# hanalice/Distributed-ResNet-Tensorflow

Measured on AMD Instinct MI355X. Metric: images/sec (whole node) ResNet-50 bs=128/GPU, higher is better.
Workload: dtype bf16; 1 GPU; model=resnet50_v2_imagenet, global_batch=128, per_gpu_batch=128, image_size=224, num_classes=1001, parallelism=dp1, hip_graph=False, step_mode=plan, wgrad_side_stream=True, fused_stem_pool=True, hw_queues=4

## Files before the change

### csrc/kernels/bn.hip

```cpp
#include "drn_common.h"
#include "drn_conv.h"
#include <stdlib.h>

namespace drn {

__global__ __launch_bounds__(256) void bn_stats_kernel(const bf16_t* __restrict__ x, float* __restrict__ part, int M,
                                                       int C, int rows_per_block, int rep) {
  extern __shared__ __attribute__((aligned(16))) char smem[];
  const int CV = C / 8;
  const int tid = threadIdx.x;
  const int rpp = 256 / CV;
  const int cv = tid % CV;
  const int r0 = tid / CV;
  float s[8], q[8];
#pragma unroll
  for (int j = 0; j < 8; ++j) s[j] = q[j] = 0.f;
  const int mbeg = blockIdx.x * rows_per_block;
  const int mend = min(M, mbeg + rows_per_block);
  if (r0 < rpp) {
    for (int m = mbeg + r0; m < mend; m += rpp) {
      const uint4 v = *reinterpret_cast<const uint4*>(x + (size_t)m * C + cv * 8);
      float f[8];
      unpack8(v, f);
#pragma unroll
// ... 486 lines not shown
    for (int j = 0; j < 8; ++j) {
      f0[j] = f0[j] * sc[j] + sh[j];
      f1[j] = f1[j] * sc[j] + sh[j];
      if (relu) {
        f0[j] = fmaxf(f0[j], 0.f);
        f1[j] = fmaxf(f1[j], 0.f);
      }
    }
    yv[i] = pack8(f0);
    yv[i + stride] = pack8(f1);
  }
  if (i < nvec) {
    float f0[8];
    unpack8(xv[i], f0);
#pragma unroll
    for (int j = 0; j < 8; ++j) {
      f0[j] = f0[j] * sc[j] + sh[j];
      if (relu) f0[j] = fmaxf(f0[j], 0.f);
    }
    yv[i] = pack8(f0);
  }
}

template <bool ADD, bool POOL>
__global__ __launch_bounds__(256) void bn_bwd_apply_fin_kernel(DySrc src, const bf16_t* __restrict__ x,
                                                               const float* __restrict__ scale,
                                                               const float* __restrict__ shift, DrnBnFin f,
                                                               const bf16_t* __restrict__ add, bf16_t* __restrict__ dx,
                                                               int64_t nvec, int C, int relu) {
  extern __shared__ __attribute__((aligned(16))) float lsm[];
  bn_bwd_apply_body<ADD, true, POOL>(src, x, scale, shift, nullptr, nullptr, nullptr, f, add, dx, nvec, C, relu, lsm);
}

static inline int grid_for(int64_t nvec, int per_thread = 1, int cap = 2048) {
  int64_t b = (nvec + 256 * per_thread - 1) / (256 * per_thread);
  if (b > cap) b = cap;
  if (b < 1) b = 1;
  return (int)b;
}

}

static bool pow2(int v) { return v > 0 && (v & (v - 1)) == 0; }

DRN_API int drn_bn_stats_blocks(int M, int C, int rows_per_block) { return (M + rows_per_block - 1) / rows_per_block; }

DRN_API int drn_bn_stats(const void* x, float* part, int M, int C, int rows_per_block, int rep, hipStream_t s) {
  if (C % 8 || C / 8 > 256 || rep < 1) return (int)hipErrorInvalidValue;
  const int G = (M + rows_per_block - 1) / rows_per_block;
  drn::launch(drn::bn_stats_kernel, dim3(G), dim3(256), 256 * 17 * 4, s, (const bf16_t*)x, part, M, C,
                     rows_per_block, rep);
  return (int)hipGetLastError();
}

DRN_API int drn_bn_finalize(float* part, int G, int C, float count, const float* gamma, const float* beta,
                            float eps, float momentum, float* run_mean, float* run_var, float* scale, float* shift,
                            float* mean, float* invstd, hipStream_t s) {
  drn::launch(drn::bn_finalize_kernel, dim3((C + 63) / 64), dim3(256), 0, s, part, G, C, count, gamma, beta,
                     eps, momentum, run_mean, run_var, scale, shift, mean, invstd);
  return (int)hipGetLastError();
}

DRN_API int drn_bn_inference_params(int C, const float* gamma, const float* beta, const float* run_mean,
                                    const float* run_var, float eps, float* scale, float* shift, float* mean,
                                    float* invstd, hipStream_t s) {
  drn::launch(drn::bn_inference_params_kernel, dim3((C + 255) / 256), dim3(256), 0, s, C, gamma, beta,
// ... 41 lines not shown
  if (C % 8 || C / 8 > 256 || rep < 1) return (int)hipErrorInvalidValue;
  const int G = (M + rows_per_block - 1) / rows_per_block;
  drn::DySrc src{(const bf16_t*)dy, dpool, pool_hw};
  drn::launch(drn::bn_bwd_reduce_kernel, dim3(G), dim3(256), 256 * 17 * 4, s, src, (const bf16_t*)x, scale,
                     shift, mean, invstd, part, M, C, rows_per_block, relu, rep);
  return (int)hipGetLastError();
}

DRN_API int drn_bn_finalize_bwd(float* part, int G, int C, float count, const float* gamma,
                                const float* invstd, float* dgamma, float* dbeta, float* coef, hipStream_t s) {
  drn::launch(drn::bn_finalize_bwd_kernel, dim3((C + 63) / 64), dim3(256), 0, s, part, G, C, count, gamma,
                     invstd, dgamma, dbeta, coef);
  return (int)hipGetLastError();
}

static bool fin_ok(const DrnBnFin* f, int C) {
  return f != nullptr && f->stats != nullptr && f->G >= 1 && f->G <= DRN_BN_FIN_GMAX && f->C == C &&
         f->count > 0.f && f->gamma != nullptr;
}

DRN_API int drn_bn_fin_fwd_launch(const DrnBnFin* f, hipStream_t s) {
  if (!fin_ok(f, f ? f->C : 0) || f->beta == nullptr || f->scale == nullptr || f->shift == nullptr ||
      f->mean == nullptr || f->invstd == nullptr)
    return (int)hipErrorInvalidValue;
  drn::launch(drn::bn_fin_fwd_kernel, dim3((f->C + 255) / 256), dim3(256), 0, s, *f);
  return (int)hipGetLastError();
}

DRN_API int drn_bn_apply_fin(const void* x, void* y, const DrnBnFin* f, int64_t M, int C, int relu, hipStream_t s) {
  if (C % 8 || !pow2(C / 8) || C / 8 > 256 || !fin_ok(f, C) || f->beta == nullptr ||
      (f->publish && (f->scale == nullptr || f->shift == nullptr || f->mean == nullptr || f->invstd == nullptr)))
    return (int)hipErrorInvalidValue;
  const int64_t nvec = M * (C / 8);
  drn::launch(drn::bn_apply_fin_kernel, dim3(drn::grid_for(nvec, 2)), dim3(256), 2 * C * sizeof(float), s,
                     (const bf16_t*)x, (bf16_t*)y, *f, nvec, C / 8, relu);
  return (int)hipGetLastError();
}

DRN_API int drn_bn_bwd_apply_fin(const void* dy, const float* dpool, int pool_hw, const void* x, const float* scale,
                                 const float* shift, const DrnBnFin* f, const void* add, void* dx, int64_t M, int C,
                                 int relu, hipStream_t s) {
  if (C % 8 || !pow2(C / 8) || C / 8 > 256 || !fin_ok(f, C) || f->mean == nullptr || f->invstd == nullptr ||
      (f->publish && (f->dgamma == nullptr || f->dbeta == nullptr)))
    return (int)hipErrorInvalidValue;
  const int64_t nvec = M * (C / 8);
  if (nvec >= (int64_t(1) << 31)) return (int)hipErrorInvalidValue;
  drn::DySrc src{(const bf16_t*)dy, dpool, pool_hw};
  const dim3 grid(drn::grid_for(nvec, 4, 1024));
  const size_t lds = 3 * C * sizeof(float);
#define DRN_BWD_FIN(ADD, POOL)                                                                                     \
  drn::launch((drn::bn_bwd_apply_fin_kernel<ADD, POOL>), grid, dim3(256), lds, s, src, (const bf16_t*)x, scale, \
                     shift, *f, (const bf16_t*)add, (bf16_t*)dx, nvec, C, relu)
  if (pool_hw > 0) {
    if (add != nullptr) DRN_BWD_FIN(true, true);
    else DRN_BWD_FIN(false, true);
  } else {
    if (add != nullptr) DRN_BWD_FIN(true, false);
    else DRN_BWD_FIN(false, false);
  }
#undef DRN_BWD_FIN
  return (int)hipGetLastError();
}

DRN_API int drn_bn_fin_size() { return (int)sizeof(DrnBnFin); }
DRN_API int drn_conv_args_size() { return (int)sizeof(DrnConvFwdArgs); }
DRN_API int drn_wgrad_args_size() { return (int)sizeof(DrnConvWgradArgs); }

DRN_API int drn_bn_bwd_apply(const void* dy, const float* dpool, int pool_hw, const void* x, const float* scale,
                             const float* shift, const float* mean, const float* invstd, const float* coef,
                             const void* add, void* dx, int64_t M, int C, int relu, hipStream_t s) {
  if (C % 8 || !pow2(C / 8) || C / 8 > 256) return (int)hipErrorInvalidValue;
  const int64_t nvec = M * (C / 8);
  if (nvec >= (int64_t(1) << 31)) return (int)hipErrorInvalidValue;
  drn::DySrc src{(const bf16_t*)dy, dpool, pool_hw};
  const dim3 grid(drn::grid_for(nvec, 4, 1024));
#define DRN_BWD(ADD, POOL)                                                                                         \
  drn::launch((drn::bn_bwd_apply_kernel<ADD, POOL>), grid, dim3(256), 0, s, src, (const bf16_t*)x, scale, shift, \
                     mean, invstd, coef, (const bf16_t*)add, (bf16_t*)dx, nvec, C, relu)
  if (pool_hw > 0) {
    if (add != nullptr) DRN_BWD(true, true);
    else DRN_BWD(false, true);
  } else {
    if (add != nullptr) DRN_BWD(true, false);
    else DRN_BWD(false, false);
  }
// ... 4 lines not shown
```

### csrc/kernels/head.hip

```cpp
#include "drn_common.h"

namespace drn {

__global__ __launch_bounds__(256) void bnrelu_pool_kernel(const bf16_t* __restrict__ x, const float* __restrict__ scale,
                                                          const float* __restrict__ shift, float* __restrict__ pooled,
                                                          int HW, int C, int relu) {
  const int n = blockIdx.x;
  const int CV = C / 8;
  for (int cv = threadIdx.x; cv < CV; cv += blockDim.x) {
    const int c = cv * 8;
    float acc[8], sc[8], sh[8];
#pragma unroll
    for (int j = 0; j < 8; ++j) {
      acc[j] = 0.f;
      sc[j] = scale ? scale[c + j] : 1.f;
      sh[j] = scale ? shift[c + j] : 0.f;
    }
    for (int hw = 0; hw < HW; ++hw) {
      float f[8];
      unpack8(*reinterpret_cast<const uint4*>(x + ((size_t)n * HW + hw) * C + c), f);
#pragma unroll
      for (int j = 0; j < 8; ++j) {
        float v = f[j] * sc[j] + sh[j];
        if (relu) v = fmaxf(v, 0.f);
        acc[j] += v;
      }
    }
    const float inv = 1.f / (float)HW;
#pragma unroll
    for (int j = 0; j < 8; ++j) pooled[(size_t)n * C + c + j] = acc[j] * inv;
  }
}

__global__ __launch_bounds__(256) void sgemm_kernel(int ta, int tb, int M, int N, int K, float alpha,
                                                    const float* __restrict__ A, int lda,
                                                    const float* __restrict__ B, int ldb, float beta,
                                                    float* __restrict__ Cm, int ldc, const float* __restrict__ bias) {
  constexpr int BM = 64, BN = 64, BK = 32;
  constexpr int LA = BK * BM / 256, LB = BK * BN / 256;
  __shared__ float As[2][BK][BM + 1];
  __shared__ float Bs[2][BK][BN + 1];
  const int tid = threadIdx.x, lane = tid & 63, wave = tid >> 6;
  const int m0 = blockIdx.y * BM, n0 = blockIdx.x * BN;
  const int wm = (wave & 1) * 32, wn = (wave >> 1) * 32;
  const int ksz = (((K + gridDim.z - 1) / gridDim.z) + BK - 1) / BK * BK;
  const int kb = blockIdx.z * ksz, ke = min(K, kb + ksz);
  if (gridDim.z > 1) {
    Cm += (size_t)blockIdx.z * M * ldc;
    beta = 0.f;
    bias = nullptr;
    alpha = 1.f;
  }
  f32x4_t acc[2][2];
#pragma unroll
  for (int i = 0; i < 2; ++i)
#pragma unroll
// ... 331 lines not shown
  const int cl = threadIdx.x & 31, sl = threadIdx.x >> 5;
  const int j = blockIdx.x * 32 + cl;
  float s0 = 0.f, s1 = 0.f, s2 = 0.f, s3 = 0.f;
  if (j < cols) {
    int n = sl;
    for (; n + 24 < rows; n += 32) {
      s0 += in[(size_t)n * cols + j];
      s1 += in[(size_t)(n + 8) * cols + j];
      s2 += in[(size_t)(n + 16) * cols + j];
      s3 += in[(size_t)(n + 24) * cols + j];
    }
    for (; n < rows; n += 8) s0 += in[(size_t)n * cols + j];
  }
  red[sl][cl] = (s0 + s1) + (s2 + s3);
  __syncthreads();
  if (sl == 0 && j < cols) {
    float s = 0.f;
#pragma unroll
    for (int k = 0; k < 8; ++k) s += red[k][cl];
    out[j] = accumulate ? out[j] + scale * s : scale * s;
  }
}

}

DRN_API int drn_bnrelu_pool(const void* x, const float* scale, const float* shift, float* pooled, int N, int HW,
                            int C, int relu, hipStream_t s) {
  if (C % 8) return (int)hipErrorInvalidValue;
  drn::launch(drn::bnrelu_pool_kernel, dim3(N), dim3(256), 0, s, (const bf16_t*)x, scale, shift, pooled, HW, C,
                     relu);
  return (int)hipGetLastError();
}

DRN_API int drn_sgemm(int ta, int tb, int M, int N, int K, float alpha, const float* A, int lda, const float* B,
                      int ldb, float beta, float* C, int ldc, const float* bias, int splits, float* ws,
                      hipStream_t s) {
  if (splits < 1 || (splits > 1 && ws == nullptr)) return (int)hipErrorInvalidValue;
  dim3 grid((N + 63) / 64, (M + 63) / 64, splits);
  drn::launch(drn::sgemm_kernel, grid, dim3(256), 0, s, ta, tb, M, N, K, alpha, A, lda, B, ldb, beta,
                     splits > 1 ? ws : C, ldc, bias);
  if (splits > 1)
    drn::launch(drn::sgemm_finish_kernel, dim3((M * N + 255) / 256), dim3(256), 0, s, ws, splits, M, N, ldc,
                       alpha, beta, C, bias);
  return (int)hipGetLastError();
}

DRN_API int drn_softmax_xent(const float* logits, const int* labels, int N, int ncls, float grad_scale,
                             float* dlogits, float* loss, float* probs, int* correct, hipStream_t s) {
  drn::launch(drn::softmax_xent_kernel, dim3(N), dim3(256), 0, s, logits, labels, ncls, grad_scale, dlogits,
                     loss, probs, correct);
  return (int)hipGetLastError();
}

DRN_API int drn_softmax_xent_ex(const float* logits, const int* labels, int N, int ncls, float grad_scale,
                                float smoothing, int top_k, float* dlogits, float* loss, float* probs, int* correct,
                                int* correct_k, hipStream_t s) {
  if (!(smoothing >= 0.f && smoothing < 1.f) || top_k < 1 || N < 1 || ncls < 1) return (int)hipErrorInvalidValue;
  auto kern = ncls <= 256 * drn::XENT_REG_ROW ? drn::softmax_xent_ex_kernel<true> : drn::softmax_xent_ex_kernel<false>;
  drn::launch(kern, dim3(N), dim3(256), 0, s, logits, labels, ncls, grad_scale, smoothing, top_k, dlogits, loss,
                     probs, correct, correct_k);
  return (int)hipGetLastError();
}

DRN_API int drn_softmax_xent_mix(const float* logits, const int* labels, const void* table, int N, int ncls,
                                 float grad_scale, float smoothing, int top_k, float* dlogits, float* loss,
                                 float* probs, int* correct, int* correct_k, hipStream_t s) {
// ... 14 lines not shown
```

### distributed_resnet_tensorflow_amd/ops/_lib.py

```python
from __future__ import annotations

import ctypes
import os
import threading
from pathlib import Path

import torch

_LIB = None
_LOCK = threading.Lock()
LIB_PATH = Path(os.environ.get("DRN_KERNEL_LIB") or Path(__file__).resolve().parent / "libdrn_kernels.so")
_OPTIONAL = {"drn_conv_trace_set", "drn_wgrad_trace_set"}

c_int = ctypes.c_int
c_i64 = ctypes.c_int64
c_f = ctypes.c_float
c_p = ctypes.c_void_p


class DrnFastDiv(ctypes.Structure):
    _fields_ = [("d", ctypes.c_uint32), ("m", ctypes.c_uint32), ("s", ctypes.c_uint32), ("pad_", ctypes.c_uint32)]

    @classmethod
    def make(cls, d: int) -> "DrnFastDiv":
# ... 47 lines not shown


def conv_cfg_info(cfg: int):
    info = DrnConvCfgInfo()
    return info if lib().drn_conv_cfg_info(int(cfg), ctypes.byref(info)) == 0 else None


_SIGS = {
    "drn_version": ([], c_int),
    "drn_conv_fwd": ([ctypes.POINTER(DrnConvFwdArgs), c_p], c_int),
    "drn_conv_fwd_tiles_p": ([c_int, c_int], c_int),
    "drn_conv_fwd2": ([ctypes.POINTER(DrnConvFwdArgs), c_p, c_p], c_int),
    "drn_conv_glds_ok": ([ctypes.POINTER(DrnConvFwdArgs)], c_int),
    "drn_conv_glds_num_cfgs": ([], c_int),
    "drn_conv_trace_set": ([c_p], c_int),
    "drn_wgrad_trace_set": ([c_p], c_int),
    "drn_conv_glds_default_cfg": ([ctypes.POINTER(DrnConvFwdArgs)], c_int),
    "drn_conv_wgrad": ([ctypes.POINTER(DrnConvWgradArgs), c_p], c_int),
    "drn_conv_wgrad2": ([ctypes.POINTER(DrnConvWgradArgs), c_p, c_int, c_p], c_int),
    "drn_splitk_reduce": ([c_p, c_p, c_i64, c_int, c_f, c_int, c_p], c_int),
    "drn_bn_stats": ([c_p, c_p, c_int, c_int, c_int, c_int, c_p], c_int),
    "drn_bn_finalize": ([c_p, c_int, c_int, c_f, c_p, c_p, c_f, c_f, c_p, c_p, c_p, c_p, c_p, c_p, c_p], c_int),
    "drn_bn_inference_params": ([c_int, c_p, c_p, c_p, c_p, c_f, c_p, c_p, c_p, c_p, c_p], c_int),
    "drn_bn_apply": ([c_p, c_p, c_p, c_p, c_i64, c_int, c_int, c_p], c_int),
    "drn_bn_apply_stats": ([c_p, c_p, c_p, c_f, c_p, c_p, c_f, c_f, c_p, c_p, c_p, c_p, c_p, c_p, c_i64, c_int,
                            c_int, c_p], c_int),
    "drn_bn_bwd_apply_stats": ([c_p, c_p, c_int, c_p, c_p, c_p, c_p, c_p, c_p, c_f, c_p, c_p, c_p, c_p, c_p, c_i64,
                                c_int, c_int, c_p], c_int),
    "drn_bn_bwd_reduce": ([c_p, c_p, c_int, c_p, c_p, c_p, c_p, c_p, c_p, c_int, c_int, c_int, c_int, c_int, c_p],
                          c_int),
    "drn_bn_finalize_bwd": ([c_p, c_int, c_int, c_f, c_p, c_p, c_p, c_p, c_p, c_p], c_int),
    "drn_bn_bwd_apply": ([c_p, c_p, c_int, c_p, c_p, c_p, c_p, c_p, c_p, c_p, c_p, c_i64, c_int, c_int, c_p], c_int),
    "drn_bnrelu_pool": ([c_p, c_p, c_p, c_p, c_int, c_int, c_int, c_int, c_p], c_int),
    "drn_sgemm": ([c_int, c_int, c_int, c_int, c_int, c_f, c_p, c_int, c_p, c_int, c_f, c_p, c_int, c_p, c_int, c_p,
                   c_p], c_int),
    "drn_softmax_xent": ([c_p, c_p, c_int, c_int, c_f, c_p, c_p, c_p, c_p, c_p], c_int),
    "drn_softmax_xent_ex": ([c_p, c_p, c_int, c_int, c_f, c_f, c_int, c_p, c_p, c_p, c_p, c_p, c_p], c_int),
    "drn_softmax_xent_mix": ([c_p, c_p, c_p, c_int, c_int, c_f, c_f, c_int, c_p, c_p, c_p, c_p, c_p, c_p], c_int),
    "drn_mix_pairs": ([c_p, c_p, c_p, c_int, c_int, c_int, c_p], c_int),
    "drn_mix_rec_size": ([], c_int),
    "drn_colsum": ([c_p, c_int, c_int, c_p, c_f, c_int, c_p], c_int),
    "drn_maxpool_fwd": ([c_p, c_p, c_p] + [c_int] * 10 + [c_p, c_int, c_p], c_int),
    "drn_maxpool_bwd": ([c_p, c_p, c_p] + [c_int] * 10 + [c_p], c_int),
    "drn_sgd_momentum": ([c_p, c_p, c_p, c_int, c_p, c_i64, c_p, c_f, c_f, c_f, c_p, c_p], c_int),
    "drn_lars_momentum": ([c_p, c_p, c_p, c_int, c_p, c_p, c_int, c_int, c_p, c_p, c_p, c_f, c_f, c_f, c_f, c_f,
                           c_p, c_p], c_int),
    "drn_sgd_momentum_ema": ([c_p, c_p, c_p, c_int, c_p, c_i64, c_p, c_f, c_f, c_f, c_p, c_p, c_p, c_p], c_int),
    "drn_lars_momentum_ema": ([c_p, c_p, c_p, c_int, c_p, c_p, c_int, c_int, c_p, c_p, c_p, c_f, c_f, c_f, c_f, c_f,
                               c_p, c_p, c_p, c_p], c_int),
    "drn_lars_slot_size": ([], c_int),
    "drn_lars_chunk": ([], c_int),
    "drn_cast_bf16": ([c_p, c_p, c_i64, c_p], c_int),
    "drn_stem_pack_input": ([c_p, c_p, c_int, c_int, c_p], c_int),
    "drn_stem_pack_weights": ([c_p, c_p, c_int, c_int, c_int, c_int, c_int, c_int, c_p], c_int),
    "drn_stem_unpack_grad": ([c_p, c_p, c_int, c_int, c_int, c_int, c_int, c_int, c_p], c_int),
    "drn_stem_conv_pool": ([c_p, c_p, c_p, c_p, c_p] + [c_int] * 11 + [c_p], c_int),
    "drn_weight_tflip": ([c_p, c_p, c_p, c_int, c_i64, c_p], c_int),
    "drn_fill_f32": ([c_p, c_i64, c_f, c_p], c_int),
    "drn_cifar_augment": ([c_p, c_p, c_p, c_int, c_int, c_int, c_int, c_p], c_int),
    "drn_vgg_preprocess": ([c_p, c_p, c_p, c_int, c_int, c_int, c_f, c_f, c_f, c_p], c_int),
    "drn_p2p_signal": ([c_p, c_int, c_p], c_int),
    "drn_p2p_reduce": ([c_p, c_int, c_int, c_p], c_int),
    "drn_p2p_reduce2": ([c_p, c_int, c_int, c_p], c_int),
    "drn_p2p_step": ([c_p, c_p, c_p], c_int),
    "drn_p2p_cast": ([c_p, c_p, c_i64, c_p], c_int),
    "drn_p2p_args_size": ([], c_int),
# ... 91 lines not shown
```

### distributed_resnet_tensorflow_amd/ops/backend.py

```python
from __future__ import annotations

import ctypes
import os
from dataclasses import dataclass
from typing import Optional

import numpy as np
import torch
import torch.nn.functional as F

from . import _lib


@dataclass(frozen=True)
class ConvGeom:
    stride: int = 1
    pad_h: int = 0
    pad_w: int = 0
    dil: int = 1


def _ptr(t):
    return None if t is None else t.data_ptr()

# ... 170 lines not shown
    @staticmethod
    def conv_stats_tiles(M, K):
        return 1

    def bn_apply_stats(self, x, y, acc, count, gamma, beta, run_mean, run_var, scale, shift, mean, invstd,
                       momentum, eps, relu=True):
        self.bn_finalize(acc.clone(), 1, count, gamma, beta, run_mean, run_var, scale, shift, mean, invstd,
                         momentum, eps, update_running=True)
        self.bn_apply(x, y, scale, shift, relu=relu)

    def bn_bwd_apply_stats(self, dy, dpool, pool_hw, x, scale, shift, mean, invstd, acc, count, gamma, dgamma,
                           dbeta, add, dx, coef, relu=True):
        self.bn_finalize_bwd(acc.clone(), 1, count, gamma, invstd, dgamma, dbeta, coef)
        self.bn_bwd_apply(dy, dpool, pool_hw, x, scale, shift, mean, invstd, coef, add, dx, relu=relu)


    def fill_(self, t, v: float):
        t.fill_(v)

    @staticmethod
    def _check_out_fill(y, residual, out_map, bn_bwd):
        assert out_map is not None and bn_bwd is None and residual is None, "out_fill: plain strided output only"
        assert out_map.P * out_map.stride >= y.shape[1] and out_map.Q * out_map.stride >= y.shape[2], \
            "out_fill: the phase grid's sibling positions do not cover the output"

    def _publish_fwd(self, f: BnCfin):
        self.bn_finalize(f.stats, f.G, f.count, f.gamma, f.beta, f.run_mean, f.run_var, f.scale, f.shift, f.mean,
                         f.invstd, f.momentum, f.eps, update_running=f.run_mean is not None)

    def bn_apply_fin(self, x, y, fin: BnCfin, relu=True):
        if fin.publish:
            self._publish_fwd(fin)
        self.bn_apply(x, y, fin.scale, fin.shift, relu=relu)

    def bn_bwd_apply_fin(self, dy, dpool, pool_hw, x, scale, shift, fin: BnCfin, add, dx, relu=True):
        C = fin.C
        coef = torch.empty(3 * C, dtype=fin.gamma.dtype, device=x.device)
        dg = fin.dgamma if fin.publish else torch.empty_like(fin.gamma)
        db = fin.dbeta if fin.publish else torch.empty_like(fin.gamma)
        self.bn_finalize_bwd(fin.stats, fin.G, fin.count, fin.gamma, fin.invstd, dg, db, coef)
        self.bn_bwd_apply(dy, dpool, pool_hw, x, scale, shift, fin.mean, fin.invstd, coef, add, dx, relu=relu)


WGRAD_PIPELINES = "0,2,3,4,5,6,7,8,9,10"


class HipBackend(_Common):
    name = "hip"
    act_dtype = torch.bfloat16
    acc_dtype = torch.float32
    stats_replicas = 8

    def __init__(self, device="cuda"):
        self.device = torch.device(device)
        self.L = _lib.lib()
        self.zero_page = torch.zeros(1024, dtype=torch.float32, device=self.device)
        self.conv_cfg: dict = {}
        self.ks_ws = torch.zeros(1, dtype=torch.float32, device=self.device)
        self.ks_tickets = torch.zeros(1 << 16, dtype=torch.int32, device=self.device)
        self.KS_FACTORS = (2, 3, 4)
        self.SK_BLOCKS = (256, 512)
        self.forced_cfg = None
        self.autotune = os.environ.get("DRN_AUTOTUNE", "1") == "1"
        self.wgrad_ns: dict = {}
        self.wgrad_atomic_ok = False
        self.wgrad_atomic_used = False
        self.forced_wgrad_ns = None
        self.tune_log: list = []
        self._db = None
        self.db_hits = 0
        self.tune_iters = int(os.environ.get("DRN_TUNE_ITERS", "5"))
        self.tune_top = int(os.environ.get("DRN_TUNE_TOP", "4"))
        self.tune_rounds = int(os.environ.get("DRN_TUNE_ROUNDS", "2"))
        self._fin_bufs: dict = {}
        self.conv_cands: dict = {}
        self._insitu = None
        self.recording = False

    def _timed(self, launch, n: int) -> float:
        ev0, ev1 = torch.cuda.Event(enable_timing=True), torch.cuda.Event(enable_timing=True)
        ev0.record()
        for _ in range(n):
            launch()
        ev1.record()
        ev1.synchronize()
        return ev0.elapsed_time(ev1) / n

    def tune_db(self):
        if self._db is None:
            from .tunedb import TuneDB, section_for
            self._db = TuneDB(section_for(self.device, self.L))
        return self._db

    def save_tune_db(self) -> bool:
        return self._db is not None and self._db.save()

    def stream(self):
        return torch.cuda.current_stream(self.device).cuda_stream

    def conv_args(self, x, w, y, g: ConvGeom, in_bn=None, relu_in=True, residual=None, stats=None, out_map=None,
                  bn_bwd=None, bn_fin: Optional[BnFin] = None, in_fin: Optional[BnCfin] = None):
        N, H, W, C = x.shape
        K, R, S, C2 = w.shape
        N2, P, Q, K2 = y.shape
        oH, oW = P, Q
        if out_map is not None:
            P, Q = out_map.P, out_map.Q
# ... 365 lines not shown
    def bn_inference(self, gamma, beta, run_mean, run_var, eps, scale, shift, mean=None, invstd=None):
        _lib.check(self.L.drn_bn_inference_params(gamma.numel(), gamma.data_ptr(), beta.data_ptr(),
                                                  run_mean.data_ptr(), run_var.data_ptr(), eps, scale.data_ptr(),
                                                  shift.data_ptr(), _ptr(mean), _ptr(invstd), self.stream()),
                   "drn_bn_inference_params")

    def bn_apply(self, x, y, scale, shift, relu=True):
        C = x.shape[-1]
        _lib.check(self.L.drn_bn_apply(x.data_ptr(), y.data_ptr(), scale.data_ptr(), shift.data_ptr(),
                                       x.numel() // C, C, 1 if relu else 0, self.stream()), "drn_bn_apply")

    def bn_apply_stats(self, x, y, acc, count, gamma, beta, run_mean, run_var, scale, shift, mean, invstd,
                       momentum, eps, relu=True):
        C = x.shape[-1]
        _aligned16(acc, gamma, beta, run_mean, run_var, scale, shift, mean, invstd)
        _lib.check(self.L.drn_bn_apply_stats(x.data_ptr(), y.data_ptr(), acc.data_ptr(), float(count),
                                             gamma.data_ptr(), beta.data_ptr(), float(eps), float(momentum),
                                             run_mean.data_ptr(), run_var.data_ptr(), scale.data_ptr(),
                                             shift.data_ptr(), mean.data_ptr(), invstd.data_ptr(), x.numel() // C, C,
                                             1 if relu else 0, self.stream()), "drn_bn_apply_stats")

    def bn_bwd_apply_stats(self, dy, dpool, pool_hw, x, scale, shift, mean, invstd, acc, count, gamma, dgamma,
                           dbeta, add, dx, coef=None, relu=True):
        C = x.shape[-1]
        _aligned16(acc, gamma, dgamma, dbeta, scale, shift, mean, invstd)
        _lib.check(self.L.drn_bn_bwd_apply_stats(_ptr(dy), _ptr(dpool), pool_hw, x.data_ptr(), scale.data_ptr(),
                                                 shift.data_ptr(), mean.data_ptr(), invstd.data_ptr(),
                                                 acc.data_ptr(), float(count), gamma.data_ptr(), dgamma.data_ptr(),
                                                 dbeta.data_ptr(), _ptr(add), dx.data_ptr(), x.numel() // C, C,
                                                 1 if relu else 0, self.stream()), "drn_bn_bwd_apply_stats")

    def bn_apply_fin(self, x, y, fin: BnCfin, relu=True):
        C = x.shape[-1]
        if C >= self.BN_FIN_SPLIT_C and fin.publish:
            self.bn_finalize(fin.stats, fin.G, fin.count, fin.gamma, fin.beta, fin.run_mean, fin.run_var, fin.scale,
                             fin.shift, fin.mean, fin.invstd, fin.momentum, fin.eps,
                             update_running=fin.run_mean is not None)
            self.bn_apply(x, y, fin.scale, fin.shift, relu=relu)
            return
        f = fin.struct()
        _lib.check(self.L.drn_bn_apply_fin(x.data_ptr(), y.data_ptr(), ctypes.byref(f), x.numel() // C, C,
                                           1 if relu else 0, self.stream()), "drn_bn_apply_fin")

    BN_FIN_SPLIT_C = 1024

    def _fin_scratch(self, C: int) -> torch.Tensor:
        buf = self._fin_bufs.get(C)
        if buf is None:
            buf = self._fin_bufs[C] = torch.empty(5 * C, dtype=torch.float32, device=self.device)
        return buf

    def bn_bwd_apply_fin(self, dy, dpool, pool_hw, x, scale, shift, fin: BnCfin, add, dx, relu=True):
        C = x.shape[-1]
        _aligned16(scale, shift)
        if C >= self.BN_FIN_SPLIT_C:
            buf = self._fin_scratch(C)
            coef = buf[:3 * C]
            dg = fin.dgamma if fin.publish else buf[3 * C:4 * C]
            db = fin.dbeta if fin.publish else buf[4 * C:]
            self.bn_finalize_bwd(fin.stats, fin.G, fin.count, fin.gamma, fin.invstd, dg, db, coef)
            self.bn_bwd_apply(dy, dpool, pool_hw, x, scale, shift, fin.mean, fin.invstd, coef, add, dx, relu=relu)
            return
        f = fin.struct()
        _lib.check(self.L.drn_bn_bwd_apply_fin(_ptr(dy), _ptr(dpool), pool_hw, x.data_ptr(), scale.data_ptr(),
                                               shift.data_ptr(), ctypes.byref(f), _ptr(add), dx.data_ptr(),
                                               x.numel() // C, C, 1 if relu else 0, self.stream()),
                   "drn_bn_bwd_apply_fin")

    def bn_bwd_reduce(self, dy, dpool, pool_hw, x, scale, shift, mean, invstd, part, relu=True):
        C = x.shape[-1]
        M = x.numel() // C
        rpb = self.bn_rows_per_block(M, C)
        _lib.check(self.L.drn_bn_bwd_reduce(_ptr(dy), _ptr(dpool), pool_hw, x.data_ptr(), scale.data_ptr(),
                                            shift.data_ptr(), mean.data_ptr(), invstd.data_ptr(), part.data_ptr(),
                                            M, C, rpb, 1 if relu else 0, part.numel() // (2 * C), self.stream()),
                   "drn_bn_bwd_reduce")
        return part.numel() // (2 * C)

    def bn_finalize_bwd(self, part, G, count, gamma, invstd, dgamma, dbeta, coef):
        _lib.check(self.L.drn_bn_finalize_bwd(part.data_ptr(), G, gamma.numel(), float(count), gamma.data_ptr(),
                                              invstd.data_ptr(), dgamma.data_ptr(), dbeta.data_ptr(),
                                              coef.data_ptr(), self.stream()), "drn_bn_finalize_bwd")

    def bn_bwd_apply(self, dy, dpool, pool_hw, x, scale, shift, mean, invstd, coef, add, dx, relu=True):
        C = x.shape[-1]
        _lib.check(self.L.drn_bn_bwd_apply(_ptr(dy), _ptr(dpool), pool_hw, x.data_ptr(), scale.data_ptr(),
                                           shift.data_ptr(), mean.data_ptr(), invstd.data_ptr(), coef.data_ptr(),
                                           _ptr(add), dx.data_ptr(), x.numel() // C, C, 1 if relu else 0,
                                           self.stream()), "drn_bn_bwd_apply")

    def pool_bnrelu(self, x, scale, shift, pooled, relu=True):
        N, H, W, C = x.shape
        _lib.check(self.L.drn_bnrelu_pool(x.data_ptr(), _ptr(scale), _ptr(shift), pooled.data_ptr(), N, H * W, C,
                                          1 if relu else 0, self.stream()), "drn_bnrelu_pool")

    _sgemm_ws: dict = {}
    _retired_ws: list = []
    SGEMM_TARGET_WG = 256

    def sgemm(self, ta, tb, M, N, K, alpha, A, lda, B, ldb, beta, C, ldc, bias=None):
        tiles = ((M + 63) // 64) * ((N + 63) // 64)
        splits = max(1, min(K // 128, self.SGEMM_TARGET_WG // max(tiles, 1)))
        ws = None
        if splits > 1:
            need = splits * M * ldc
            key = (C.device, self.stream())
            ws = HipBackend._sgemm_ws.get(key)
            if ws is None or ws.numel() < need:
                if ws is not None:
                    if torch.cuda.is_current_stream_capturing():
                        raise RuntimeError("sgemm workspace must be sized before graph capture")
                    HipBackend._retired_ws.append(ws)
                ws = torch.empty(max(need, 1 << 20), dtype=torch.float32, device=C.device)
                HipBackend._sgemm_ws[key] = ws
        _lib.check(self.L.drn_sgemm(int(ta), int(tb), M, N, K, float(alpha), A.data_ptr(), lda, B.data_ptr(), ldb,
                                    float(beta), C.data_ptr(), ldc, _ptr(bias), splits, _ptr(ws), self.stream()),
                   "drn_sgemm")

    def softmax_xent(self, logits, labels, grad_scale, dlogits, loss, correct, probs=None):
        N, ncls = logits.shape
        _lib.check(self.L.drn_softmax_xent(logits.data_ptr(), labels.data_ptr(), N, ncls, float(grad_scale),
                                           _ptr(dlogits), loss.data_ptr(), _ptr(probs), _ptr(correct),
                                           self.stream()), "drn_softmax_xent")

    def softmax_xent_ex(self, logits, labels, grad_scale, dlogits, loss, correct, probs=None, smoothing=0.0, top_k=1,
                        correct_k=None):
        N, ncls = logits.shape
# ... 599 lines not shown
```

### distributed_resnet_tensorflow_amd/runtime/executor.py

```python
from __future__ import annotations

import contextlib
import os

from dataclasses import dataclass
from typing import Callable, List, Optional

import torch

from ..models.spec import Block, BN, Conv, NetSpec
from ..ops.backend import BnCfin, ConvGeom, OutMap, dgrad_geom, tflip_desc, tflip_table
from .params import ParamStore

BN_DECAY = 0.997
BN_EPSILON = 1e-5


@dataclass
class BNState:
    bn: BN
    gamma: torch.Tensor
    beta: torch.Tensor
    dgamma: torch.Tensor
    dbeta: torch.Tensor
# ... 154 lines not shown
                        Hph = (in_hw - ph + st - 1) // st
                        Wph = (in_hw - pw + st - 1) // st
                        if not rs or not ss or Hph <= 0 or Wph <= 0:
                            full = False
                            continue
                        r0, s0 = max(rs), max(ss)
                        dmin_h, dmin_w = (ph + p - r0) // st, (pw + p - s0) // st
                        wt_descs.append(tflip_desc(s.offset, wt_off, K, R, R, C, Ru=len(rs), Sv=len(ss),
                                                   r0=r0, s0=s0, dr=-st, ds=-st))
                        phases.append(DgradPhase((C, len(rs), len(ss), K), wt_off,
                                                 ConvGeom(1, -dmin_h, -dmin_w, 1), OutMap(Hph, Wph, st, ph, pw)))
                        wt_off += C * len(rs) * len(ss) * K
        op = ConvOp(c, g, P.compute_w(name), phases, P.g(name), s.offset, full)
        return op, wt_off

    def _bn_shapes(self):
        sp, N = self.spec, self.N
        hs = sp.stem_hw
        out = [(N * hs * hs, sp.stem.cout)]
        if sp.maxpool:
            out.append((N * sp.pool_hw * sp.pool_hw, sp.stem.cout))
        for blk in sp.blocks:
            hw = blk.in_hw
            out.append((N * hw * hw, blk.in_c))
            for b, c in zip(blk.bns, blk.convs[:-1]):
                hw = c.out_hw(hw)
                out += [(N * hw * hw, c.cout)] * 2
            out.append((N * blk.out_hw * blk.out_hw, blk.out_c))
        out.append((N * sp.blocks[-1].out_hw ** 2, sp.final_c))
        return out

    def _det_replicas(self, M: int, C: int) -> int:
        return max(((M + 63) // 64) * ((C + 63) // 64), 1024)

    def _reps(self, C: int) -> int:
        r = max(1, min(self.stats_rep, self.stats_rep * 256 // C))
        return min(r, 8) if self.cfin else r

    def _stats_for(self, M: int, C: int) -> tuple[torch.Tensor, int]:
        R = self._det_replicas(M, C) if self.deterministic else self._reps(C)
        n = (2 * C * R + 15) // 16 * 16
        if self._arena_off + n > self._arena_cap:
            raise RuntimeError("statistics arena exhausted")
        t = self.stats_arena[self._arena_off:self._arena_off + 2 * C * R].view(R, 2, C)
        self._arena_off += n
        return t, R

    def all_bn_states(self) -> List[BNState]:
        return [b for bp in self.blocks for b in bp.bn] + [self.final_bn]

    def _alloc(self):
        sp, N = self.spec, self.N
        be = self.be
        all_c = [b.c for blk in sp.blocks for b in [blk.bn1] + list(blk.bns)] + [sp.final_bn.c, sp.stem.cout]
        self.stats_rep = int(getattr(be, "stats_replicas", 1))
        if self.deterministic:
            arena = 64 + sum(2 * ((2 * c * self._det_replicas(m, c) + 15) // 16 * 16) for m, c in self._bn_shapes())
        else:
            arena = sum(2 * ((2 * c * self._reps(c) + 15) // 16 * 16) for c in all_c) + 64
        self._arena_cap = arena
        self.stats_arena = self._f32(arena)
        self._arena_off = 0
        wt_descs, wt_off = [], 0
        self.stem_op, wt_off = self._conv_op(sp.stem, wt_descs, wt_off)
        self._stem_hi = int(self.stem_op.dw.numel()) if self.stem_op.grad_lo == 0 else 0
        stem_macs = N * sp.stem_hw * sp.stem_hw * sp.stem.cout * sp.stem.k * sp.stem.k * sp.stem.cin_store
# ... 222 lines not shown

    def forward(self, train: bool = True):
        be, sp = self.be, self.spec
        if train:
            be.zero_(self.stats_arena)
        st = self.stem_op
        if self.stem_pool:
            be.stem_pack_input(self.images, self.stem_xp)
            fused = train and not self.deterministic
            img = sp.image_size
            be.stem_conv_pool(self.stem_xp, self.stem_w4, self.pool_out, self.pool_arg, self.stem_geom4, img, img,
                              sp.stem_hw, sp.stem_hw, stats=self.pool_stats if fused else None)
            if train and not fused:
                be.bn_stats(self.pool_out, self.pool_stats)
        elif self.stem_pack:
            be.stem_pack_input(self.images, self.stem_xp)
            be.conv_fwd(self.stem_xp, self.stem_w4, self.stem_out, self.stem_geom4,
                        stats=self.stem_stats if train else None)
        else:
            be.conv_fwd(self.images, st.w, self.stem_out, st.geom, stats=self.stem_stats if train else None)
        if sp.maxpool and not self.stem_pool:
            ph = sp.pool_hw
            pad = max((ph - 1) * 2 + 3 - sp.stem_hw, 0) // 2
            fused = train and not self.deterministic
            be.maxpool_fwd(self.stem_out, self.pool_out, self.pool_arg, 3, 2, pad, pad,
                           stats=self.pool_stats if fused else None)
            if train and not fused:
                be.bn_stats(self.pool_out, self.pool_stats)
        for bp in self.blocks:
            self._block_fwd(bp, train)
            if self.check_nan:
                self._check(bp.out, f"forward output of block {bp.blk.stage}.{bp.blk.index}")
        fb = self.final_bn
        self._bn_fwd(fb, train)
        be.pool_bnrelu(self.last_out, fb.scale, fb.shift, self.pooled, relu=True)
        N, C, ncls = self.N, sp.final_c, sp.num_classes
        be.sgemm(0, 1, N, ncls, C, 1.0, self.pooled, C, self.dense_w, C, 0.0, self.logits, ncls, bias=self.dense_b)
        smoothing = self.label_smoothing if train else 0.0
        if self.mix and train:
            be.softmax_xent_mix(self.logits, self.labels, self.mix_table, 1.0 / N, self.dlogits, self.loss_vec,
                                self.correct, smoothing=smoothing, top_k=max(self.top_k, 1),
                                correct_k=self.correct_k)
        elif smoothing == 0.0 and self.top_k < 2:
            be.softmax_xent(self.logits, self.labels, 1.0 / N, self.dlogits if train else None, self.loss_vec,
                            self.correct)
        else:
            be.softmax_xent_ex(self.logits, self.labels, 1.0 / N, self.dlogits if train else None, self.loss_vec,
                               self.correct, smoothing=smoothing, top_k=max(self.top_k, 1),
                               correct_k=self.correct_k)
        if self.check_nan:
            self._check(self.loss_vec, "cross-entropy")

    def set_mix(self, table):
        if self.mix_table is None:
            raise RuntimeError("this executor does not mix (Executor(mix=False))")
        from ..ops.backend import mix_table_tensor
        t = mix_table_tensor(table)
        if tuple(t.shape) != (self.N, 8):
            raise ValueError(f"the mix table has {t.shape[0]} records, the batch {self.N} samples")
        self.mix_table.copy_(t, non_blocking=True)

    def _check(self, t: torch.Tensor, what: str):
        if not bool(torch.isfinite(t.float()).all()):
            raise FloatingPointError(f"non-finite values in {what}")

    def check_gradients(self):
        bad = [s.name for s in self.P.slots
               if not bool(torch.isfinite(self.P.grad[s.offset:s.offset + s.numel]).all())]
# ... 407 lines not shown
```

Before: 13350 images/sec.

## Slice fused BN-finalize kernels by channel and fuse finalize into final pool

Adds channel-sliced variants of the fused BN-finalize apply and backward-apply kernels for C>256. Each block finalizes only a 256-channel slice in shared memory, so wide layers no longer go through separate finalize and apply launches. Also fuses the final BN's finalize into the global-average-pool+ReLU head kernel, removing a separate BN forward step. The trade-off is redundant finalize work across blocks: every row-block recomputes the statistics reduction for its slice, and the pool kernel recomputes it per image.

```diff
diff --git a/csrc/kernels/bn.hip b/csrc/kernels/bn.hip
--- a/csrc/kernels/bn.hip
+++ b/csrc/kernels/bn.hip
@@ -542,6 +542,138 @@
   bn_bwd_apply_body<ADD, true, POOL>(src, x, scale, shift, nullptr, nullptr, nullptr, f, add, dx, nvec, C, relu, lsm);
 }
 
+constexpr int kFinSlice = 256;
+
+struct BnSlice {
+  uint32_t i0, stride;
+  int c0, cl;
+};
+__device__ __forceinline__ BnSlice bn_slice(int C) {
+  constexpr int SV = kFinSlice / 8, ROWS = 256 / SV;
+  const int CV = C / 8;
+  const int sv = threadIdx.x % SV, r = threadIdx.x / SV;
+  BnSlice s;
+  s.c0 = blockIdx.y * kFinSlice;
+  s.cl = sv * 8;
+  s.i0 = (blockIdx.x * ROWS + r) * CV + blockIdx.y * SV + sv;
+  s.stride = gridDim.x * ROWS * CV;
+  return s;
+}
+
+__global__ __launch_bounds__(256) void bn_apply_fin_sliced_kernel(const bf16_t* __restrict__ x,
+                                                                  bf16_t* __restrict__ y, DrnBnFin f, int64_t nvec,
+                                                                  int CV, int relu) {
+  __shared__ __attribute__((aligned(16))) float lsm[2 * kFinSlice];
+  const BnSlice sl = bn_slice(CV * 8);
+  {
+    const int t = fin_slot(threadIdx.x);
+    drn_bn_fin_fwd(f, sl.c0 + threadIdx.x, f.publish && blockIdx.x == 0, lsm[t], lsm[kFinSlice + t]);
+  }
+  __syncthreads();
+  float sc[8], sh[8];
+  load8f_fin(lsm, sl.cl, sc);
+  load8f_fin(lsm + kFinSlice, sl.cl, sh);
+  const int64_t stride = sl.stride;
+  const uint4* xv = reinterpret_cast<const uint4*>(x);
+  uint4* yv = reinterpret_cast<uint4*>(y);
+  int64_t i = sl.i0;
+  for (; i + stride < nvec; i += 2 * stride) {
+    const uint4 v0 = xv[i], v1 = xv[i + stride];
+    float f0[8], f1[8];
+    unpack8(v0, f0);
+    unpack8(v1, f1);
+#pragma unroll
+    for (int j = 0; j < 8; ++j) {
+      f0[j] = f0[j] * sc[j] + sh[j];
+      f1[j] = f1[j] * sc[j] + sh[j];
+      if (relu) {
+        f0[j] = fmaxf(f0[j], 0.f);
+        f1[j] = fmaxf(f1[j], 0.f);
+      }
+    }
+    yv[i] = pack8(f0);
+    yv[i + stride] = pack8(f1);
+  }
+  if (i < nvec) {
+    float f0[8];
+    unpack8(xv[i], f0);
+#pragma unroll
+    for (int j = 0; j < 8; ++j) {
+      f0[j] = f0[j] * sc[j] + sh[j];
+      if (relu) f0[j] = fmaxf(f0[j], 0.f);
+    }
+    yv[i] = pack8(f0);
+  }
+}
+
+template <bool ADD, bool POOL>
+__global__ __launch_bounds__(256) void bn_bwd_apply_fin_sliced_kernel(DySrc src, const bf16_t* __restrict__ x,
+                                                                      const float* __restrict__ scale,
+                                                                      const float* __restrict__ shift, DrnBnFin f,
+                                                                      const bf16_t* __restrict__ add,
+                                                                      bf16_t* __restrict__ dx, int64_t nvec, int C,
+                                                                      int relu) {
+  __shared__ __attribute__((aligned(16))) float lsm[3 * kFinSlice];
+  constexpr int U = 4;
+  const int cv_shift = __ffs(C / 8) - 1;
+  const uint32_t n = (uint32_t)nvec;
+  const BnSlice sl = bn_slice(C);
+  const uint32_t stride = sl.stride, i0 = sl.i0;
+  const int c = sl.c0 + sl.cl;
+  const uint4* __restrict__ xg = reinterpret_cast<const uint4*>(x);
+  const uint4* __restrict__ dg = reinterpret_cast<const uint4*>(src.dy);
+  const uint4* __restrict__ ag = reinterpret_cast<const uint4*>(add);
+  uint4* __restrict__ og = reinterpret_cast<uint4*>(dx);
+  const uint32_t safe = i0 < n ? i0 : 0;
+  uint4 xr[U], dr[U], ar[U];
+  auto load = [&](uint32_t base) {
+#pragma unroll
+    for (int u = 0; u < U; ++u) {
+      const uint32_t i = base + u * stride < n ? base + u * stride : safe;
+      xr[u] = xg[i];
+      if constexpr (!POOL) dr[u] = dg[i];
+      if constexpr (ADD) ar[u] = ag[i];
+    }
+  };
+  load(i0);
+  float sc[8], sh[8], A[8], B[8], D[8];
+  load8f(scale + c, sc);
+  load8f(shift + c, sh);
+  {
+    const int t = fin_slot(threadIdx.x);
+    drn_bn_fin_bwd(f, sl.c0 + threadIdx.x, f.publish && blockIdx.x == 0, lsm[t], lsm[kFinSlice + t],
+                   lsm[2 * kFinSlice + t]);
+  }
+  __syncthreads();
+  load8f_fin(lsm, sl.cl, A);
+  load8f_fin(lsm + kFinSlice, sl.cl, B);
+  load8f_fin(lsm + 2 * kFinSlice, sl.cl, D);
+  for (uint32_t base = i0; base < n; base += U * stride) {
+    uint4 o[U];
+#pragma unroll
+    for (int u = 0; u < U; ++u) {
+      float fd[8];
+      if constexpr (POOL) src.load_vec(base + u * stride < n ? base + u * stride : safe, cv_shift, C, c, fd);
+      else unpack8(dr[u], fd);
+      bn_bwd_fin_vec<ADD>(xr[u], fd, ar[u], A, B, D, sc, sh, relu);
+      o[u] = pack8(fd);
+    }
+#pragma unroll
+    for (int u = 0; u < U; ++u)
+      if (base + u * stride < n) og[base + u * stride] = o[u];
+    if (base + U * stride < n) load(base + U * stride);
+  }
+}
+
+static inline dim3 sliced_grid(int64_t M, int C, int per_thread, int cap) {
+  const int gy = C / kFinSlice;
+  const int rows = 256 / (kFinSlice / 8) * per_thread;
+  int64_t gx = (M + rows - 1) / rows;
+  if (gx > cap / gy) gx = cap / gy;
+  if (gx < 1) gx = 1;
+  return dim3((unsigned)gx, (unsigned)gy);
+}
+
 static inline int grid_for(int64_t nvec, int per_thread = 1, int cap = 2048) {
   int64_t b = (nvec + 256 * per_thread - 1) / (256 * per_thread);
   if (b > cap) b = cap;
@@ -649,6 +781,12 @@
       (f->publish && (f->scale == nullptr || f->shift == nullptr || f->mean == nullptr || f->invstd == nullptr)))
     return (int)hipErrorInvalidValue;
   const int64_t nvec = M * (C / 8);
+  if (C > drn::kFinSlice) {
+    if (nvec >= (int64_t(1) << 31)) return (int)hipErrorInvalidValue;
+    drn::launch(drn::bn_apply_fin_sliced_kernel, drn::sliced_grid(M, C, 2, 2048), dim3(256), 0, s, (const bf16_t*)x,
+                (bf16_t*)y, *f, nvec, C / 8, relu);
+    return (int)hipGetLastError();
+  }
   drn::launch(drn::bn_apply_fin_kernel, dim3(drn::grid_for(nvec, 2)), dim3(256), 2 * C * sizeof(float), s,
                      (const bf16_t*)x, (bf16_t*)y, *f, nvec, C / 8, relu);
   return (int)hipGetLastError();
@@ -665,9 +803,17 @@
   drn::DySrc src{(const bf16_t*)dy, dpool, pool_hw};
   const dim3 grid(drn::grid_for(nvec, 4, 1024));
   const size_t lds = 3 * C * sizeof(float);
+  const bool sliced = C > drn::kFinSlice;
+  const dim3 sgrid = sliced ? drn::sliced_grid(M, C, 4, 1024) : grid;
 #define DRN_BWD_FIN(ADD, POOL)                                                                                     \
-  drn::launch((drn::bn_bwd_apply_fin_kernel<ADD, POOL>), grid, dim3(256), lds, s, src, (const bf16_t*)x, scale, \
-                     shift, *f, (const bf16_t*)add, (bf16_t*)dx, nvec, C, relu)
+  do {                                                                                                             \
+    if (sliced)                                                                                                    \
+      drn::launch((drn::bn_bwd_apply_fin_sliced_kernel<ADD, POOL>), sgrid, dim3(256), 0, s, src,                  \
+                  (const bf16_t*)x, scale, shift, *f, (const bf16_t*)add, (bf16_t*)dx, nvec, C, relu);             \
+    else                                                                                                           \
+      drn::launch((drn::bn_bwd_apply_fin_kernel<ADD, POOL>), grid, dim3(256), lds, s, src, (const bf16_t*)x,      \
+                  scale, shift, *f, (const bf16_t*)add, (bf16_t*)dx, nvec, C, relu);                               \
+  } while (0)
   if (pool_hw > 0) {
     if (add != nullptr) DRN_BWD_FIN(true, true);
     else DRN_BWD_FIN(false, true);
diff --git a/csrc/kernels/head.hip b/csrc/kernels/head.hip
--- a/csrc/kernels/head.hip
+++ b/csrc/kernels/head.hip
@@ -1,4 +1,5 @@
 #include "drn_common.h"
+#include "drn_conv.h"
 
 namespace drn {
 
@@ -22,6 +23,35 @@
 #pragma unroll
       for (int j = 0; j < 8; ++j) {
         float v = f[j] * sc[j] + sh[j];
+        if (relu) v = fmaxf(v, 0.f);
+        acc[j] += v;
+      }
+    }
+    const float inv = 1.f / (float)HW;
+#pragma unroll
+    for (int j = 0; j < 8; ++j) pooled[(size_t)n * C + c + j] = acc[j] * inv;
+  }
+}
+
+__global__ __launch_bounds__(256) void bnrelu_pool_fin_kernel(const bf16_t* __restrict__ x, DrnBnFin f,
+                                                              float* __restrict__ pooled, int HW, int C, int relu) {
+  const int n = blockIdx.x;
+  const int CV = C / 8;
+  const bool pub = f.publish && blockIdx.x == 0;
+  for (int cv = threadIdx.x; cv < CV; cv += blockDim.x) {
+    const int c = cv * 8;
+    float acc[8], sc[8], sh[8];
+#pragma unroll
+    for (int j = 0; j < 8; ++j) {
+      acc[j] = 0.f;
+      drn_bn_fin_fwd(f, c + j, pub, sc[j], sh[j]);
+    }
+    for (int hw = 0; hw < HW; ++hw) {
+      float v8[8];
+      unpack8(*reinterpret_cast<const uint4*>(x + ((size_t)n * HW + hw) * C + c), v8);
+#pragma unroll
+      for (int j = 0; j < 8; ++j) {
+        float v = v8[j] * sc[j] + sh[j];
         if (relu) v = fmaxf(v, 0.f);
         acc[j] += v;
       }
@@ -419,6 +449,16 @@
   return (int)hipGetLastError();
 }
 
+DRN_API int drn_bnrelu_pool_fin(const void* x, const DrnBnFin* f, float* pooled, int N, int HW, int C, int relu,
+                                hipStream_t s) {
+  if (C % 8 || N < 1 || f == nullptr || f->stats == nullptr || f->G < 1 || f->G > DRN_BN_FIN_GMAX || f->C != C ||
+      !(f->count > 0.f) || f->gamma == nullptr || f->beta == nullptr ||
+      (f->publish && (f->scale == nullptr || f->shift == nullptr || f->mean == nullptr || f->invstd == nullptr)))
+    return (int)hipErrorInvalidValue;
+  drn::launch(drn::bnrelu_pool_fin_kernel, dim3(N), dim3(256), 0, s, (const bf16_t*)x, *f, pooled, HW, C, relu);
+  return (int)hipGetLastError();
+}
+
 DRN_API int drn_sgemm(int ta, int tb, int M, int N, int K, float alpha, const float* A, int lda, const float* B,
                       int ldb, float beta, float* C, int ldc, const float* bias, int splits, float* ws,
                       hipStream_t s) {
diff --git a/distributed_resnet_tensorflow_amd/ops/_lib.py b/distributed_resnet_tensorflow_amd/ops/_lib.py
--- a/distributed_resnet_tensorflow_amd/ops/_lib.py
+++ b/distributed_resnet_tensorflow_amd/ops/_lib.py
@@ -103,6 +103,7 @@
     "drn_bn_finalize_bwd": ([c_p, c_int, c_int, c_f, c_p, c_p, c_p, c_p, c_p, c_p], c_int),
     "drn_bn_bwd_apply": ([c_p, c_p, c_int, c_p, c_p, c_p, c_p, c_p, c_p, c_p, c_p, c_i64, c_int, c_int, c_p], c_int),
     "drn_bnrelu_pool": ([c_p, c_p, c_p, c_p, c_int, c_int, c_int, c_int, c_p], c_int),
+    "drn_bnrelu_pool_fin": ([c_p, c_p, c_p, c_int, c_int, c_int, c_int, c_p], c_int),
     "drn_sgemm": ([c_int, c_int, c_int, c_int, c_int, c_f, c_p, c_int, c_p, c_int, c_f, c_p, c_int, c_p, c_int, c_p,
                    c_p], c_int),
     "drn_softmax_xent": ([c_p, c_p, c_int, c_int, c_f, c_p, c_p, c_p, c_p, c_p], c_int),
diff --git a/distributed_resnet_tensorflow_amd/ops/backend.py b/distributed_resnet_tensorflow_amd/ops/backend.py
--- a/distributed_resnet_tensorflow_amd/ops/backend.py
+++ b/distributed_resnet_tensorflow_amd/ops/backend.py
@@ -226,6 +226,11 @@
         if fin.publish:
             self._publish_fwd(fin)
         self.bn_apply(x, y, fin.scale, fin.shift, relu=relu)
+
+    def pool_bnrelu_fin(self, x, fin: BnCfin, pooled, relu=True):
+        if fin.publish:
+            self._publish_fwd(fin)
+        self.pool_bnrelu(x, fin.scale, fin.shift, pooled, relu=relu)
 
     def bn_bwd_apply_fin(self, dy, dpool, pool_hw, x, scale, shift, fin: BnCfin, add, dx, relu=True):
         C = fin.C
@@ -266,7 +271,6 @@
         self.tune_iters = int(os.environ.get("DRN_TUNE_ITERS", "5"))
         self.tune_top = int(os.environ.get("DRN_TUNE_TOP", "4"))
         self.tune_rounds = int(os.environ.get("DRN_TUNE_ROUNDS", "2"))
-        self._fin_bufs: dict = {}
         self.conv_cands: dict = {}
         self._insitu = None
         self.recording = False
@@ -698,35 +702,15 @@
 
     def bn_apply_fin(self, x, y, fin: BnCfin, relu=True):
         C = x.shape[-1]
-        if C >= self.BN_FIN_SPLIT_C and fin.publish:
-            self.bn_finalize(fin.stats, fin.G, fin.count, fin.gamma, fin.beta, fin.run_mean, fin.run_var, fin.scale,
-                             fin.shift, fin.mean, fin.invstd, fin.momentum, fin.eps,
-                             update_running=fin.run_mean is not None)
-            self.bn_apply(x, y, fin.scale, fin.shift, relu=relu)
-            return
         f = fin.struct()
         _lib.check(self.L.drn_bn_apply_fin(x.data_ptr(), y.data_ptr(), ctypes.byref(f), x.numel() // C, C,
                                            1 if relu else 0, self.stream()), "drn_bn_apply_fin")
 
-    BN_FIN_SPLIT_C = 1024
-
-    def _fin_scratch(self, C: int) -> torch.Tensor:
-        buf = self._fin_bufs.get(C)
-        if buf is None:
-            buf = self._fin_bufs[C] = torch.empty(5 * C, dtype=torch.float32, device=self.device)
-        return buf
+    BN_FIN_SPLIT_C = 1 << 30
 
     def bn_bwd_apply_fin(self, dy, dpool, pool_hw, x, scale, shift, fin: BnCfin, add, dx, relu=True):
         C = x.shape[-1]
         _aligned16(scale, shift)
-        if C >= self.BN_FIN_SPLIT_C:
-            buf = self._fin_scratch(C)
-            coef = buf[:3 * C]
-            dg = fin.dgamma if fin.publish else buf[3 * C:4 * C]
-            db = fin.dbeta if fin.publish else buf[4 * C:]
-            self.bn_finalize_bwd(fin.stats, fin.G, fin.count, fin.gamma, fin.invstd, dg, db, coef)
-            self.bn_bwd_apply(dy, dpool, pool_hw, x, scale, shift, fin.mean, fin.invstd, coef, add, dx, relu=relu)
-            return
         f = fin.struct()
         _lib.check(self.L.drn_bn_bwd_apply_fin(_ptr(dy), _ptr(dpool), pool_hw, x.data_ptr(), scale.data_ptr(),
                                                shift.data_ptr(), ctypes.byref(f), _ptr(add), dx.data_ptr(),
@@ -759,6 +743,12 @@
         N, H, W, C = x.shape
         _lib.check(self.L.drn_bnrelu_pool(x.data_ptr(), _ptr(scale), _ptr(shift), pooled.data_ptr(), N, H * W, C,
                                           1 if relu else 0, self.stream()), "drn_bnrelu_pool")
+
+    def pool_bnrelu_fin(self, x, fin: BnCfin, pooled, relu=True):
+        N, H, W, C = x.shape
+        f = fin.struct()
+        _lib.check(self.L.drn_bnrelu_pool_fin(x.data_ptr(), ctypes.byref(f), pooled.data_ptr(), N, H * W, C,
+                                              1 if relu else 0, self.stream()), "drn_bnrelu_pool_fin")
 
     _sgemm_ws: dict = {}
     _retired_ws: list = []
diff --git a/distributed_resnet_tensorflow_amd/runtime/executor.py b/distributed_resnet_tensorflow_amd/runtime/executor.py
--- a/distributed_resnet_tensorflow_amd/runtime/executor.py
+++ b/distributed_resnet_tensorflow_amd/runtime/executor.py
@@ -210,6 +210,8 @@
 
     def _det_replicas(self, M: int, C: int) -> int:
         return max(((M + 63) // 64) * ((C + 63) // 64), 1024)
+
+    POOL_FIN_MIN_C = 256
 
     def _reps(self, C: int) -> int:
         r = max(1, min(self.stats_rep, self.stats_rep * 256 // C))
@@ -498,8 +500,11 @@
             if self.check_nan:
                 self._check(bp.out, f"forward output of block {bp.blk.stage}.{bp.blk.index}")
         fb = self.final_bn
-        self._bn_fwd(fb, train)
-        be.pool_bnrelu(self.last_out, fb.scale, fb.shift, self.pooled, relu=True)
+        if train and self.cfin and fb.bn.c > self.POOL_FIN_MIN_C:
+            be.pool_bnrelu_fin(self.last_out, self._fin_fwd_spec(fb, publish=True), self.pooled, relu=True)
+        else:
+            self._bn_fwd(fb, train)
+            be.pool_bnrelu(self.last_out, fb.scale, fb.shift, self.pooled, relu=True)
         N, C, ncls = self.N, sp.final_c, sp.num_classes
         be.sgemm(0, 1, N, ncls, C, 1.0, self.pooled, C, self.dense_w, C, 0.0, self.logits, ncls, bias=self.dense_b)
         smoothing = self.label_smoothing if train else 0.0
```

Result: no change. 13470 images/sec, median of 6 (+0.9%).
